# navallo/collision_avoidance

Measured on NVIDIA B200. Metric: orca_agent_steps_per_sec, higher is better.
Workload: dtype f32

## Files before the change

collision_avoidance_b200/build.py:

```python
from __future__ import annotations

import os
import shutil
import subprocess
import sys

PKG_DIR = os.path.dirname(os.path.abspath(__file__))
CSRC = os.path.join(PKG_DIR, "csrc")
LIB_PATH = os.path.join(PKG_DIR, "liborca_b200.so")

NVCC_FLAGS = [
    "-O3", "-std=c++17",
    "-gencode", "arch=compute_100a,code=sm_100a",
    "-lineinfo",
    "-fmad=false",
    "-Xcompiler", "-fPIC,-ffp-contract=off,-O2",
    "-shared",
]


def _sources_mtime() -> float:
    newest = 0.0
    for root in (CSRC, os.path.join(PKG_DIR, "..", "include")):
        for name in os.listdir(root):
            if name.endswith((".cu", ".cuh", ".h")):
                newest = max(newest, os.path.getmtime(os.path.join(root, name)))
    return newest


def nvcc_path() -> str:
    nvcc = shutil.which("nvcc") or "/usr/local/cuda/bin/nvcc"
    if not os.path.exists(nvcc):
        raise RuntimeError("nvcc not found: the CUDA library cannot be built")
    return nvcc


def build(force: bool = False, verbose: bool = False, extra_flags=()) -> str:
    if not force and os.path.exists(LIB_PATH) and os.path.getmtime(LIB_PATH) >= _sources_mtime():
        return LIB_PATH
    cmd = [nvcc_path(), *NVCC_FLAGS, *extra_flags, "-o", LIB_PATH, os.path.join(CSRC, "orca_api.cu")]
    if verbose:
        print(" ".join(cmd), file=sys.stderr)
    subprocess.check_call(cmd)
    return LIB_PATH


if __name__ == "__main__":
    flags = [a for a in sys.argv[1:] if a != "-v"]
    print(build(force=True, verbose=True, extra_flags=flags))
```

collision_avoidance_b200/csrc/orca_core.cuh:

```cuda
#pragma once

#include <math.h>
#include <stdint.h>

#if defined(__CUDACC__)
#define ORCA_HD __host__ __device__ __forceinline__
#define ORCA_HD_NOINLINE __host__ __device__ __noinline__
#else
#define ORCA_HD inline
#define ORCA_HD_NOINLINE inline
#include "host_vec_types.h"
#endif
#include <string.h>

#ifndef ORCA_MAX_OBST_NEIGHBORS
#define ORCA_MAX_OBST_NEIGHBORS 16
#endif
#ifndef ORCA_MAX_OBST_LINES
#define ORCA_MAX_OBST_LINES 6
#endif
#ifndef ORCA_MAX_ACTIONS
#define ORCA_MAX_ACTIONS 16
#endif
#define ORCA_MAX_BSP_DEPTH 64
#ifndef ORCA_SLOW_MAX_OBST
#define ORCA_SLOW_MAX_OBST 64
#endif

#if defined(ORCA_EMUL_COUNT) && !defined(__CUDA_ARCH__)
extern long long g_orca_counters[16];
#define ORCA_COUNT(slot, n) (g_orca_counters[slot] += (n))
#else
#define ORCA_COUNT(slot, n) ((void)0)
#endif

#if defined(ORCA_DEBUG_CHECKS)
#include <assert.h>
#define ORCA_DCHECK(cond) assert(cond)
#else
#define ORCA_DCHECK(cond) ((void)0)
#endif

namespace orca {

constexpr float kEps = 0.00001f;

ORCA_HD float bits_to_float(int i) {
#if defined(__CUDA_ARCH__)
  return __int_as_float(i);
#else
  float f;
  memcpy(&f, &i, 4);
  return f;
#endif
}
ORCA_HD int float_to_bits(float f) {
#if defined(__CUDA_ARCH__)
  return __float_as_int(f);
#else
  int i;
  memcpy(&i, &f, 4);
  return i;
#endif
}

ORCA_HD float2 v2(float x, float y) {
  float2 r;
  r.x = x;
  r.y = y;
  return r;
}
ORCA_HD float2 add(float2 a, float2 b) { return v2(a.x + b.x, a.y + b.y); }
ORCA_HD float2 sub(float2 a, float2 b) { return v2(a.x - b.x, a.y - b.y); }
ORCA_HD float2 neg(float2 a) { return v2(-a.x, -a.y); }
ORCA_HD float2 mul(float s, float2 a) { return v2(s * a.x, s * a.y); }
ORCA_HD float dot(float2 a, float2 b) { return a.x * b.x + a.y * b.y; }
ORCA_HD float det(float2 a, float2 b) { return a.x * b.y - a.y * b.x; }
ORCA_HD float abs_sq(float2 a) { return a.x * a.x + a.y * a.y; }
ORCA_HD float sqr(float s) { return s * s; }
ORCA_HD float2 div_s(float2 a, float s) {
  const float inv = 1.0f / s;
  return v2(a.x * inv, a.y * inv);
}
ORCA_HD float2 unit(float2 a) { return div_s(a, sqrtf(abs_sq(a))); }
ORCA_HD float left_of(float2 a, float2 b, float2 c) { return det(sub(a, c), sub(b, a)); }
ORCA_HD float fmin_first(float a, float b) { return (b < a) ? b : a; }
ORCA_HD float fmax_first(float a, float b) { return (a < b) ? b : a; }

ORCA_HD float dist_sq_point_segment(float2 a, float2 b, float2 c) {
  const float2 ab = sub(b, a);
  const float r = dot(sub(c, a), ab) / abs_sq(ab);
  if (r < 0.f) return abs_sq(sub(c, a));
  if (r > 1.f) return abs_sq(sub(c, b));
  return abs_sq(sub(c, add(a, mul(r, ab))));
}

struct Lines {
  float4* base;
  int stride;
  ORCA_HD float4 get(int i) const { return base[i * stride]; }
  ORCA_HD bool fetch(int i, float4& out) const {
    out = base[i * stride];
    return true;
  }
  ORCA_HD void set(int i, float2 point, float2 dir) const {
    float4 v;
    v.x = point.x;
    v.y = point.y;
    v.z = dir.x;
    v.w = dir.y;
    base[i * stride] = v;
  }
};
ORCA_HD float2 pt(float4 l) { return v2(l.x, l.y); }
ORCA_HD float2 dr(float4 l) { return v2(l.z, l.w); }

#if defined(__CUDA_ARCH__)
#define ORCA_LDG(p) __ldg(p)
#else
#define ORCA_LDG(p) (*(p))
#endif

struct ObstacleWorld {
  const float4* vert_pd;
  const int4* vert_link;
  const int4* bsp;
  const float4* bsp_seg;
  int n_nodes;
  const uint32_t* cull_rows;
  float4 cull_geo;
};

ORCA_HD bool obstacles_may_be_near(const ObstacleWorld& W, float2 p) {
  if (W.cull_rows == nullptr) return true;
  const float fx = (p.x - W.cull_geo.x) * W.cull_geo.z, fy = (p.y - W.cull_geo.y) * W.cull_geo.w;
  if (!(fx >= 0.f && fx < 32.f && fy >= 0.f && fy < 32.f)) return true;
  return ((ORCA_LDG(&W.cull_rows[(int)fy]) >> (int)fx) & 1u) != 0u;
}

#define ORCA_LD(p) (*(p))


template <class LS>
ORCA_HD bool lp1(const LS& S, int i, float4 li, float radius, float2 opt, bool dir_opt, float2& result) {
  const float2 pi = pt(li), di = dr(li);
  const float dp = dot(pi, di);
  const float disc = sqr(dp) + sqr(radius) - abs_sq(pi);
  if (disc < 0.f) return false;
  const float sq = sqrtf(disc);
  float t_lo = -dp - sq;
  float t_hi = -dp + sq;
  ORCA_COUNT(2, 1);
  ORCA_COUNT(3, i);
  for (int j = 0; j < i; ++j) {
    float4 lj;
    if (!S.fetch(j, lj)) continue;
    const float den = det(di, dr(lj));
    const float num = det(dr(lj), sub(pi, pt(lj)));
    if (fabsf(den) <= kEps) {
      if (num < 0.f) return false;
      continue;
    }
    const float t = num / den;
    if (den >= 0.f)
      t_hi = fmin_first(t_hi, t);
    else
      t_lo = fmax_first(t_lo, t);
    if (t_lo > t_hi) return false;
  }
  float t;
  if (dir_opt) {
    t = (dot(opt, di) > 0.f) ? t_hi : t_lo;
  } else {
    t = dot(di, sub(opt, pi));
    if (t < t_lo)
      t = t_lo;
    else if (t > t_hi)
      t = t_hi;
  }
  result = add(pi, mul(t, di));
  return true;
}

#if defined(__CUDA_ARCH__)
#define ORCA_ANY(mask, pred) __any_sync((mask), (pred))
#define ORCA_CONVERGE(mask) __syncwarp(mask)
#else
#define ORCA_ANY(mask, pred) (pred)
#define ORCA_CONVERGE(mask) ((void)0)
#endif

template <class LS>
ORCA_HD int lp2(unsigned mask, bool enabled, const LS& S, int n, float radius, float2 opt, bool dir_opt,
                float2& result) {
  if (dir_opt) {
    result = mul(radius, opt);
  } else if (abs_sq(opt) > sqr(radius)) {
    result = mul(radius, unit(opt));
  } else {
    result = opt;
  }
  int i = 0;
  int fail = n;
  bool active = enabled;
  while (ORCA_ANY(mask, active)) {
    float4 li;
    li.x = li.y = li.z = li.w = 0.f;
    if (active) {
      while (i < n) {
        if (S.fetch(i, li) && det(dr(li), sub(pt(li), result)) > 0.f) break;
        ++i;
      }
      active = i < n;
    }
    ORCA_CONVERGE(mask);
    if (active) {
      const float2 keep = result;
      if (!lp1(S, i, li, radius, opt, dir_opt, result)) {
        result = keep;
        fail = i;
        active = false;
      }
      ++i;
    }
  }
  return fail;
}

template <class LS>
struct ProjectedLines {
  LS L;
  float2 pi, di;
  int n_obst;
  ORCA_HD bool fetch(int j, float4& out) const {
    ORCA_COUNT(4, 1);
    const float4 lj = L.get(j);
    if (j < n_obst) {
      out = lj;
      return true;
    }
    const float2 pj = pt(lj), dj = dr(lj);
    const float d = det(di, dj);
    float2 np;
    if (fabsf(d) <= kEps) {
      if (dot(di, dj) > 0.f) return false;
      np = mul(0.5f, add(pi, pj));
    } else {
      np = add(pi, mul(det(dj, sub(pi, pj)) / d, di));
    }
    const float2 nd = unit(sub(dj, di));
    out.x = np.x;
    out.y = np.y;
    out.z = nd.x;
    out.w = nd.y;
    return true;
  }
};

template <class LS>
ORCA_HD void lp3(unsigned mask, bool need, const LS& L, int n, int n_obst, int begin, float radius, float2& result) {
  float distance = 0.f;
  int i = begin;
  bool active = need;
  while (ORCA_ANY(mask, active)) {
    ProjectedLines<LS> V;
    V.L = L;
    V.pi = v2(0.f, 0.f);
    V.di = v2(0.f, 0.f);
    V.n_obst = n_obst;
    if (active) {
      while (i < n) {
        const float4 li = L.get(i);
        V.pi = pt(li);
        V.di = dr(li);
        if (det(V.di, sub(V.pi, result)) > distance) break;
        ++i;
      }
      active = i < n;
      if (active) ORCA_COUNT(0, 1);
    }
    ORCA_CONVERGE(mask);
    const int m = active ? (i > n_obst ? i : n_obst) : 0;
    float2 cand = result;
    const int f = lp2(mask, active, V, m, radius, v2(-V.di.y, V.di.x), true, cand);
    if (active) {
      if (!(f < m)) result = cand;
      distance = det(V.di, sub(V.pi, result));
      ++i;
    }
  }
}

template <class LS, class PS>
ORCA_HD void lp3_stored(unsigned mask, bool need, const LS& L, int n, int n_obst, int begin, float radius, const PS& P,
                        float2& result) {
  float distance = 0.f;
  int i = begin;
  bool active = need;
  while (ORCA_ANY(mask, active)) {
    float2 pi = v2(0.f, 0.f), di = v2(0.f, 0.f);
    if (active) {
      while (i < n) {
        const float4 li = L.get(i);
        pi = pt(li);
        di = dr(li);
        if (det(di, sub(pi, result)) > distance) break;
        ++i;
      }
      active = i < n;
    }
    ORCA_CONVERGE(mask);
    int m = 0;
    if (active) {
      ProjectedLines<LS> V;
      V.L = L;
      V.pi = pi;
      V.di = di;
      V.n_obst = n_obst;
      const int hi = i > n_obst ? i : n_obst;
      for (int j = 0; j < hi; ++j) {
        float4 lj;
        if (V.fetch(j, lj)) P.set(m++, pt(lj), dr(lj));
      }
    }
    ORCA_CONVERGE(mask);
    float2 cand = result;
    const int f = lp2(mask, active, P, m, radius, v2(-di.y, di.x), true, cand);
    if (active) {
      if (!(f < m)) result = cand;
      distance = det(di, sub(pi, result));
      ++i;
    }
  }
}

ORCA_HD float4 agent_line(float2 p, float2 v, float2 po, float2 vo, float cr, float inv_th, float inv_dt,
                          bool* collided) {
  const float2 rp = sub(po, p);
  const float2 rv = sub(v, vo);
  const float d_sq = abs_sq(rp);
  const float cr_sq = sqr(cr);
  const bool apart = d_sq > cr_sq;
  const float inv_t = apart ? inv_th : inv_dt;
  const float2 w = sub(rv, mul(inv_t, rp));
  const float w_sq = abs_sq(w);
  const float dp1 = dot(w, rp);
  const bool on_circle = !apart || (dp1 < 0.f && sqr(dp1) > cr_sq * w_sq);
  const float root = sqrtf(on_circle ? w_sq : (d_sq - cr_sq));
  const float inv = 1.0f / (on_circle ? root : d_sq);
  float2 dir, u;
  if (on_circle) {
    const float2 uw = v2(w.x * inv, w.y * inv);
    dir = v2(uw.y, -uw.x);
    u = mul(cr * inv_t - root, uw);
  } else {
    const float leg = root;
    if (det(rp, w) > 0.f) {
      dir = v2((rp.x * leg - rp.y * cr) * inv, (rp.x * cr + rp.y * leg) * inv);
    } else {
      dir = neg(v2((rp.x * leg + rp.y * cr) * inv, (-rp.x * cr + rp.y * leg) * inv));
    }
    const float dp2 = dot(rv, dir);
    u = sub(mul(dp2, dir), rv);
  }
  *collided = !apart;
  const float2 point = add(v, mul(0.5f, u));
  float4 out;
  out.x = point.x;
  out.y = point.y;
  out.z = dir.x;
  out.w = dir.y;
  return out;
}

ORCA_HD unsigned lt_as_one_bits(float x, float y) {
#if defined(__CUDA_ARCH__)
  float one_or_zero;
  asm("set.lt.f32.f32 %0, %1, %2;" : "=f"(one_or_zero) : "f"(x), "f"(y));
  return __float_as_uint(one_or_zero);
#else
  return (x < y) ? 0x3f800000u : 0u;
#endif
}
ORCA_HD int one_bits_count(unsigned sum) { return (int)(((sum >> 23) * 383u) & 511u); }

template <int M>
ORCA_HD void rank_count(const float* d, int* r) {
#if defined(__CUDA_ARCH__)
  unsigned u[M];
#pragma unroll
  for (int j = 0; j < M; ++j) u[j] = (unsigned)j * 0x3f800000u;
#pragma unroll
  for (int i = 0; i < M; ++i) {
#pragma unroll
    for (int j = i + 1; j < M; ++j) {
      float j_first;
      asm("set.lt.f32.f32 %0, %1, %2;" : "=f"(j_first) : "f"(d[j]), "f"(d[i]));
      u[i] += __float_as_uint(j_first);
      u[j] -= __float_as_uint(j_first);
    }
  }
#pragma unroll
  for (int j = 0; j < M; ++j) r[j] = (int)(((u[j] >> 23) * 383u) & 511u);
#else
  for (int j = 0; j < M; ++j) r[j] = j;
  for (int i = 0; i < M; ++i) {
    for (int j = i + 1; j < M; ++j) {
      const int j_first = (d[j] < d[i]) ? 1 : 0;
      r[i] += j_first;
      r[j] -= j_first;
    }
  }
#endif
}

template <int K, bool KFULL>
struct NearestK {
  float d[K];
  int id[K];
  int k;
  float range_sq;
  uint4 packed;
  int packed_cnt;
  ORCA_HD void init(int k_, float range_sq_) {
    k = k_;
    range_sq = range_sq_;
    packed_cnt = -1;
#pragma unroll
    for (int s = 0; s < K; ++s) {
      d[s] = (KFULL || s < k) ? range_sq : -1.0f;
      id[s] = -1;
    }
  }
  ORCA_HD void set_sorted_ids(const uint4 packed_, int cnt) {
    packed = packed_;
    packed_cnt = cnt;
  }
  ORCA_HD void unpack_ids() {
#pragma unroll
    for (int s = 0; s < K; ++s) {
      const unsigned w = (s < 4) ? packed.x : (s < 8) ? packed.y : (s < 12) ? packed.z : packed.w;
      id[s] = (s < packed_cnt) ? (int)((w >> ((s & 3) * 8)) & 255u) : -1;
      d[s] = 0.f;
    }
  }
  ORCA_HD float thresh() const {
    if (KFULL) return d[K - 1];
    float m = d[0];
#pragma unroll
    for (int s = 1; s < K; ++s) m = fmaxf(m, d[s]);
    return m;
  }
  ORCA_HD void offer(float cand_d, int cand_id) {
    if (cand_d < thresh()) {
      bool prev_before = false;
      float prev_d = cand_d;
      int prev_i = cand_id;
#pragma unroll
      for (int s = 0; s < K; ++s) {
        const bool before = cand_d < d[s];
        const float old_d = d[s];
        const int old_i = id[s];
        d[s] = before ? (prev_before ? prev_d : cand_d) : old_d;
        id[s] = before ? (prev_before ? prev_i : cand_id) : old_i;
        prev_before = before;
        prev_d = old_d;
        prev_i = old_i;
      }
    }
  }
  ORCA_HD void finish() {}
  ORCA_HD bool full() const { return id[K - 1] >= 0; }
  ORCA_HD float kth_dist_sq() const { return d[K - 1]; }
  template <class Before>
  ORCA_HD void offer_ranked(float cand_d, int cand_id, const Before& precedes) {
    bool tie = false;
#pragma unroll
    for (int s = 0; s < K; ++s) tie = tie || (cand_d == d[s]);
    if (!tie) {
      offer(cand_d, cand_id);
      return;
    }
    if (cand_d <= thresh()) {
      bool prev_before = false;
      float prev_d = cand_d;
      int prev_i = cand_id;
#pragma unroll
      for (int s = 0; s < K; ++s) {
        bool before = cand_d < d[s];
        if (cand_d == d[s]) before = precedes(cand_id, id[s]);
        const float old_d = d[s];
        const int old_i = id[s];
        d[s] = before ? (prev_before ? prev_d : cand_d) : old_d;
        id[s] = before ? (prev_before ? prev_i : cand_id) : old_i;
        prev_before = before;
        prev_d = old_d;
        prev_i = old_i;
      }
    }
  }
};

template <int K, bool KFULL>
struct NearestKeys {
  unsigned long long key[K];
  int id[K];
  float d[K];
  int k;
  float range_sq;
  uint4 packed;
  int packed_cnt;
  ORCA_HD void init(int k_, float range_sq_) {
    k = k_;
    range_sq = range_sq_;
    packed_cnt = -1;
    const unsigned long long empty = (unsigned long long)(unsigned)float_to_bits(range_sq_) << 32;
#pragma unroll
    for (int s = 0; s < K; ++s) {
      key[s] = (KFULL || s < k) ? empty : 0ull;
      id[s] = -1;
      d[s] = 0.f;
    }
  }
  ORCA_HD float thresh() const {
    unsigned long long m = key[K - 1];
    if (!KFULL) {
#pragma unroll
      for (int s = 0; s < K - 1; ++s) m = key[s] > m ? key[s] : m;
    }
    return bits_to_float((int)(unsigned)(m >> 32));
  }
  ORCA_HD void offer(float cand_d, int cand_id) {
    unsigned long long x = ((unsigned long long)(unsigned)float_to_bits(cand_d) << 32) | (unsigned)(cand_id + 1);
    if (KFULL && !(x < key[K - 1])) return;
#pragma unroll
    for (int s = 0; s < K; ++s) {
      const unsigned long long cur = key[s];
      const bool in_front = x < cur;
      key[s] = in_front ? x : cur;
      x = in_front ? cur : x;
    }
  }
  template <class Before>
  ORCA_HD void offer_ranked(float cand_d, int cand_id, const Before&) {
    offer(cand_d, cand_id);
  }
  ORCA_HD void finish() {
#pragma unroll
    for (int s = 0; s < K; ++s) id[s] = (int)(unsigned)(key[s] & 0xffffffffull) - 1;
  }
  ORCA_HD bool full() const { return id[K - 1] >= 0; }
  ORCA_HD float kth_dist_sq() const { return bits_to_float((int)(unsigned)(key[K - 1] >> 32)); }
  ORCA_HD void pack_ids() {
    unsigned w[4] = {0u, 0u, 0u, 0u};
    int cnt = 0;
#pragma unroll
    for (int s = 0; s < K; ++s) {
      const bool valid = id[s] >= 0;
      w[s >> 2] |= valid ? ((unsigned)id[s] << ((s & 3) * 8)) : 0u;
      cnt += valid ? 1 : 0;
    }
    packed.x = w[0];
    packed.y = w[1];
    packed.z = w[2];
    packed.w = w[3];
    packed_cnt = cnt;
  }
  ORCA_HD void set_sorted_ids(const uint4 packed_, int cnt) {
    packed = packed_;
    packed_cnt = cnt;
  }
  ORCA_HD void unpack_ids() {
#pragma unroll
    for (int s = 0; s < K; ++s) {
      const unsigned w = (s < 4) ? packed.x : (s < 8) ? packed.y : (s < 12) ? packed.z : packed.w;
      id[s] = (s < packed_cnt) ? (int)((w >> ((s & 3) * 8)) & 255u) : -1;
    }
  }
};

#if defined(__CUDA_ARCH__)
#define ORCA_WARP_MAX(mask, v) __reduce_max_sync((mask), (v))
#else
#define ORCA_WARP_MAX(mask, v) (v)
#endif

struct CandidateBuffer {
  float4* base;
  int stride;
  int cap;
  int cnt;
  ORCA_HD float2* entry(int r) const { return reinterpret_cast<float2*>(&base[(r >> 1) * stride]) + (r & 1); }
  ORCA_HD void push(float d, int id) {
    ORCA_DCHECK(cnt >= 0 && cnt < cap);
    *entry(cnt) = v2(d, bits_to_float(id));
    ++cnt;
  }
  template <class Insert>
  ORCA_HD void drain(unsigned mask, const Insert& insert) {
    const int rounds = ORCA_WARP_MAX(mask, cnt);
    for (int r = 0; r < rounds; ++r) {
      if (r < cnt) {
        const float2 e = *entry(r);
        insert(e.x, float_to_bits(e.y));
      }
    }
    cnt = 0;
  }
  template <class Insert>
  ORCA_HD void drain_if_full(unsigned mask, const Insert& insert, int room = 1) {
    if (ORCA_ANY(mask, cnt + room > cap)) drain(mask, insert);
  }
};

template <int MAXN = ORCA_MAX_OBST_NEIGHBORS>
// ... 258 lines not shown
```

collision_avoidance_b200/csrc/orca_step_small.cuh:

```cuda
#pragma once

#include "orca_core.cuh"

namespace orca {

constexpr int kMaxDevices = 64;

enum : int { POLICY_EXTERNAL = 0, POLICY_GOAL = 1, POLICY_RL = 2, POLICY_ALAN = 3 };
enum : int { DONE_NONE = 0, DONE_GOAL_RADIUS = 1, DONE_X_BELOW = 2, DONE_GOAL_RADIUS_DEFERRED = 3 };
enum : int {
  STAT_AGENT_STEPS = 0,
  STAT_FINISHED = 1,
  STAT_COLLISIONS = 2,
  STAT_LP3_CALLS = 3,
  STAT_OVERFLOW = 4,
  STAT_SUM_ARRIVAL = 5,
  STAT_SUM_ARRIVAL2 = 6,
  STAT_SUM_REWARD = 7
};

struct StepArgs {
  int E, N, envs_per_block, env_base;
  int k;
  float dt, inv_dt, nd_sq, inv_th, inv_tho, radius, vmax, obst_range_sq;
// ... 472 lines not shown
        a.nbr_idx[(size_t)g * a.k + s] = (nk.id[s] >= 0) ? src.local_id(nk.id[s]) : -1;
        if (a.nbr_dsq != nullptr) a.nbr_dsq[(size_t)g * a.k + s] = (nk.id[s] >= 0) ? abs_sq(sub(p, src.pos(nk.id[s]))) : 0.f;
        cnt += (nk.id[s] >= 0) ? 1 : 0;
      }
    }
    a.nbr_cnt[g] = cnt;
  }
  if (a.onbr_idx != nullptr) {
    int* row = a.onbr_idx + (size_t)g * ORCA_MAX_OBST_NEIGHBORS;
    if ((reinterpret_cast<uintptr_t>(a.onbr_idx) & 15u) == 0u) {
#pragma unroll
      for (int s = 0; s < ORCA_MAX_OBST_NEIGHBORS; s += 4) {
        int4 w;
        w.x = (s + 0 < ocnt) ? oid[s + 0] : -1;
        w.y = (s + 1 < ocnt) ? oid[s + 1] : -1;
        w.z = (s + 2 < ocnt) ? oid[s + 2] : -1;
        w.w = (s + 3 < ocnt) ? oid[s + 3] : -1;
        *reinterpret_cast<int4*>(row + s) = w;
      }
    } else {
      for (int s = 0; s < ORCA_MAX_OBST_NEIGHBORS; ++s) row[s] = (s < ocnt) ? oid[s] : -1;
    }
    a.onbr_cnt[g] = ocnt;
  }
  if (a.neighbors_only) return false;

  int n_obst = 0;
  if (ocnt > 0)
    n_obst = obstacle_lines<OL>(W, p, v, HETERO ? ap.radius : a.radius, HETERO ? ap.inv_tho : a.inv_tho, od, oid, ocnt, L,
                                &overflow);
  const float inv_th = HETERO ? ap.inv_th : a.inv_th;
  int n = n_obst;
  unsigned collisions = 0;
  {
    const float cr = a.radius + a.radius;
#ifndef ORCA_UNROLLED_LINES
    if (nk.packed_cnt >= 0) {
      unsigned w0 = nk.packed.x, w1 = nk.packed.y, w2 = nk.packed.z, w3 = nk.packed.w;
      const int cnt = nk.packed_cnt;
#pragma unroll 1
      for (int s = 0; s < cnt; ++s) {
        const int j = (int)(w0 & 255u);
        w0 = (w0 >> 8) | (w1 << 24);
        w1 = (w1 >> 8) | (w2 << 24);
        w2 = (w2 >> 8) | (w3 << 24);
        w3 >>= 8;
        bool hit;
        ORCA_DCHECK(n < K + OL);
        const float4 ln = agent_line(p, v, src.pos(j), src.vel(j), HETERO ? ap.radius + src.radius(j) : cr, inv_th, a.inv_dt, &hit);
        L.base[n * L.stride] = ln;
        ++n;
        collisions += hit ? 1u : 0u;
      }
    } else {
      int ids[K + 1];
#pragma unroll
      for (int s = 0; s < K; ++s) ids[s] = nk.id[s];
      ids[K] = -1;
      int j = ids[0];
      float2 pj = v2(0.f, 0.f), vj = v2(0.f, 0.f);
      if (j >= 0) {
        pj = src.pos(j);
        vj = src.vel(j);
      }
#pragma unroll 1
      for (int s = 1; j >= 0; ++s) {
        const int jn = ids[s];
        float2 pn = pj, vn = vj;
        if (jn >= 0) {
          pn = src.pos(jn);
          vn = src.vel(jn);
        }
        bool hit;
        const float4 ln = agent_line(p, v, pj, vj, HETERO ? ap.radius + src.radius(j) : cr, inv_th, a.inv_dt, &hit);
        L.base[n * L.stride] = ln;
        ++n;
        collisions += hit ? 1u : 0u;
        j = jn;
        pj = pn;
        vj = vn;
      }
    }
#else
    {
      if (nk.packed_cnt >= 0) nk.unpack_ids();
#pragma unroll
      for (int s = 0; s < K; ++s) {
        const int j = nk.id[s];
        if (j >= 0) {
          bool hit;
          const float4 ln = agent_line(p, v, src.pos(j), src.vel(j), HETERO ? ap.radius + src.radius(j) : cr, inv_th, a.inv_dt, &hit);
          L.base[n * L.stride] = ln;
          ++n;
          collisions += hit ? 1u : 0u;
        }
      }
    }
#endif
  }
  c.n = n;
  c.n_obst = n_obst;
  c.collisions = collisions;
  c.overflow = overflow;

  c.fail = lp2(warp_mask, true, L, n, HETERO ? ap.vmax : a.vmax, pref, false, c.nv);
  return true;
}

struct SlowParams {
  int k;
  float nd_sq, inv_th, inv_tho, inv_dt, radius, vmax, obst_range_sq;
};
struct SlowResult {
  float2 nv;
  int n, n_obst, fail;
  unsigned collisions;
  bool overflow;
};
ORCA_HD SlowParams slow_params(const StepArgs& a) {
  SlowParams q;
  q.k = a.k;
  q.nd_sq = a.nd_sq;
  q.inv_th = a.inv_th;
  q.inv_tho = a.inv_tho;
  q.inv_dt = a.inv_dt;
  q.radius = a.radius;
  q.vmax = a.vmax;
  q.obst_range_sq = a.obst_range_sq;
  return q;
}
ORCA_HD SlowParams slow_params(const StepArgs& a, const float4* agent_params, const int g) {
  const AgentParams ap = load_agent_params(agent_params, g);
  SlowParams q;
  q.k = ap.k;
  q.nd_sq = ap.nd_sq;
  q.inv_th = ap.inv_th;
  q.inv_tho = ap.inv_tho;
  q.inv_dt = a.inv_dt;
  q.radius = ap.radius;
  q.vmax = ap.vmax;
  q.obst_range_sq = ap.obst_range_sq;
  return q;
}
template <int K, bool KFULL, class Src, bool HETERO = false>
ORCA_HD_NOINLINE SlowResult agent_slow_path(const SlowParams a, const Src src, const ObstacleWorld W, const Lines scratch,
                                            const int scratch_slots, const unsigned mask, const float2 p, const float2 v,
                                            const float2 pref) {
  bool overflow = false;
  float od[ORCA_SLOW_MAX_OBST];
  int oid[ORCA_SLOW_MAX_OBST];
  int ocnt = 0;
  obstacle_neighbors<ORCA_SLOW_MAX_OBST>(W, p, a.obst_range_sq, od, oid, &ocnt, &overflow);
  float4 buf[ORCA_SLOW_MAX_OBST + K];
  Lines L;
  L.base = buf;
  L.stride = 1;
  const int n_obst = obstacle_lines<ORCA_SLOW_MAX_OBST>(W, p, v, a.radius, a.inv_tho, od, oid, ocnt, L, &overflow);
  typename Src::template List<K, KFULL> nk;
  nk.init(a.k, a.nd_sq);
  src.gather(nk, p, scratch, scratch_slots, mask);
  if (nk.packed_cnt >= 0) nk.unpack_ids();
  int n = n_obst;
  unsigned collisions = 0;
  const float cr = a.radius + a.radius;
  for (int s = 0; s < K; ++s) {
    const int j = nk.id[s];
    if (j >= 0) {
      bool hit;
      buf[n++] = agent_line(p, v, src.pos(j), src.vel(j), HETERO ? a.radius + src.radius(j) : cr, a.inv_th, a.inv_dt, &hit);
      collisions += hit ? 1u : 0u;
    }
  }
  SlowResult r;
  r.n = n;
  r.n_obst = n_obst;
  r.collisions = collisions;
  r.overflow = overflow;
  r.nv = v2(0.f, 0.f);
  r.fail = lp2(mask, true, L, n, a.vmax, pref, false, r.nv);
  float2 nv = r.nv;
  lp3(mask, r.fail < n, L, n, n_obst, r.fail, a.vmax, nv);
  r.nv = nv;
  return r;
}
ORCA_HD void apply_slow_result(const SlowResult& r, AgentCarry& c) {
  c.nv = r.nv;
  c.n = r.n;
  c.n_obst = r.n_obst;
  c.fail = r.fail;
  c.collisions = r.collisions;
  c.overflow = r.overflow;
}

template <int POLICY>
ORCA_HD void agent_back(const StepArgs& a, const int env, const int la, const int g, const int estep,
                        const AgentCarry& c, const bool live = true) {
  stat_add_u64_warp(a.stats, STAT_AGENT_STEPS, live ? 1u : 0u);
  stat_add_u64_warp(a.stats, STAT_LP3_CALLS, (live && c.fail < c.n) ? 1u : 0u);

  const float2 v = c.nv;
  const float2 p = add(c.p, mul(a.dt, v));
  a.pos[g] = p;
  a.vel[g] = v;
  if (a.pos_mirror != nullptr) a.pos_mirror[g] = p;
  if (a.vel_mirror != nullptr) a.vel_mirror[g] = v;

  if (POLICY == POLICY_RL || POLICY == POLICY_ALAN) {
    const float r_goal = dot(v, c.gdir);
    const float r_polite = dot(v, c.pref);
    float R;
    if (POLICY == POLICY_RL)
      R = a.rl_scale * r_goal + (1.f - a.rl_scale) * r_polite;
    else
      R = a.alan_gamma * r_goal + (1.f - a.alan_gamma) * r_polite;
    if (a.reward != nullptr) a.reward[g] = R;
    stat_add_f64_warp(a.stats, STAT_SUM_REWARD, live ? R : 0.f);
    if (POLICY == POLICY_ALAN) {
      float* wrow = a.alan_w + (size_t)g * a.A;
      if (a.alan_window > 0 && ((estep + 1) % a.alan_window) == 0) {
        for (int i = 0; i < a.A; ++i) wrow[i] = 0.f;
      }
      wrow[c.act] = R;
    }
  }

  if (a.done_mode != DONE_NONE) {
    const uint8_t flag = a.done[g];
    if (flag == 2) {
      a.done[g] = 1;
      if (a.goal2 != nullptr) a.goal[g] = a.goal2[g];
    } else if (flag == 0) {
      bool hit;
      if (a.done_mode != DONE_X_BELOW) {
        const float2 d = sub(p, a.goal[g]);
        hit = sqrtf(abs_sq(d)) < 2.f * a.radius;
      } else {
        hit = p.x < a.done_x;
      }
      if (hit) {
        const bool defer = a.done_mode == DONE_GOAL_RADIUS_DEFERRED;
        a.done[g] = defer ? 2 : 1;
        const float t_arr = (float)(estep + 1) * a.dt;
        if (a.arrival != nullptr) a.arrival[g] = t_arr;
        if (a.goal2 != nullptr && !defer) a.goal[g] = a.goal2[g];
        if (a.env_done_cnt != nullptr) counter_inc(&a.env_done_cnt[env]);
        stat_add_u64(a.stats, STAT_FINISHED, 1ull);
        stat_add_f64(a.stats, STAT_SUM_ARRIVAL, (double)t_arr);
        stat_add_f64(a.stats, STAT_SUM_ARRIVAL2, (double)t_arr * (double)t_arr);
      }
    }
  }
  if (a.env_step != nullptr && la == 0 && !a.grid_path) a.env_step[env] = estep + 1;
  stat_add_u64_warp(a.stats, STAT_COLLISIONS, live ? c.collisions : 0u);
  stat_add_u64_warp(a.stats, STAT_OVERFLOW, c.overflow ? 1u : 0u);
}

template <int K, bool KFULL, int POLICY, bool HETERO = false, class Src>
ORCA_HD void agent_step_body(const StepArgs& a, const int env, const int la, const int g, float2 p, float2 v,
                             const int estep, const Src& src, const Lines L, const unsigned warp_mask,
                             const float4* agent_params = nullptr) {
  AgentCarry c;
  c.p = p;
  c.v = v;
  c.aim = (POLICY == POLICY_EXTERNAL) ? a.pref[g] : a.goal[g];
  const ObstacleWorld W = Src::kObstacleCull ? global_world_with_cull(a, env) : global_world(a, env);
  if (!agent_front<K, KFULL, POLICY, ORCA_MAX_OBST_LINES, HETERO>(a, env, g, estep, src, W, L, warp_mask, c, agent_params)) return;
  if (c.overflow)
    apply_slow_result(agent_slow_path<K, KFULL, Src, HETERO>(HETERO ? slow_params(a, agent_params, g) : slow_params(a), src, global_world(a, env), L,
                                                             K + ORCA_MAX_OBST_LINES, warp_mask, c.p, c.v, c.pref), c);
  else
    lp3(warp_mask, c.fail < c.n, L, c.n, c.n_obst, c.fail, HETERO ? load_agent_params(agent_params, g).vmax : a.vmax, c.nv);
  agent_back<POLICY>(a, env, la, g, estep, c);
}

#if defined(__CUDACC__)

#ifndef ORCA_STEP_MAX_THREADS
#define ORCA_STEP_MAX_THREADS 256
#endif
#ifndef ORCA_STEP_MIN_BLOCKS
#define ORCA_STEP_MIN_BLOCKS 3
#endif

#ifndef ORCA_LP3_SMEM_POOL
#define ORCA_LP3_SMEM_POOL 0
#endif
inline size_t step_smem_bytes(int K, int tpb, bool tile, int world_slots = 0, int obst_lines = ORCA_MAX_OBST_LINES,
                              bool hetero = false) {
  size_t b = (size_t)world_slots * 64 + 16;
  if (hetero) b += (size_t)tpb * (tile ? 8 : 4);
  b += (size_t)tpb * ((tile ? 16 : 0) + (size_t)(K + obst_lines) * 16 + 8 + 4 + 1) + 8 * 4;
#if ORCA_LP3_SMEM_POOL
  b += (size_t)(tpb / 2) * (K + obst_lines) * 16 + 16;
#endif
  return b;
}

#ifndef ORCA_BLOCK_LP3
#define ORCA_BLOCK_LP3 1
#endif
#ifndef ORCA_LP3_SMEM_POOL
#define ORCA_LP3_SMEM_POOL 0
#endif
template <int K, bool HETERO = false>
__device__ __forceinline__ void block_lp3(float4* s_lines, float4* s_pool, int* s_meta, float2* s_nv,
                                          unsigned char* s_queue, int* s_warp_cnt, const bool need, const AgentCarry& c, const float vmax,
                                          const bool area_was_borrowed = false, const float* s_vmax = nullptr) {
  const int tid = threadIdx.x, lane = tid & 31, warp = tid >> 5, nwarps = blockDim.x >> 5;
  if (area_was_borrowed) __syncthreads();
#if !ORCA_BLOCK_LP3
  {
    Lines L;
    L.base = s_lines + tid;
    L.stride = blockDim.x;
    float2 nv = c.nv;
    lp3(0xffffffffu, need, L, c.n, c.n_obst, c.fail, HETERO ? s_vmax[tid] : vmax, nv);
    s_nv[tid] = nv;
    __syncwarp();
    return;
  }
#endif
  s_meta[tid] = c.n | (c.n_obst << 8) | (c.fail << 16);
  s_nv[tid] = c.nv;
  const unsigned bal = __ballot_sync(0xffffffffu, need);
  if (lane == 0) s_warp_cnt[warp] = __popc(bal);
  __syncthreads();
  int offset = 0, total = 0;
  for (int w = 0; w < nwarps; ++w) {
    const int cw = s_warp_cnt[w];
    offset += (w < warp) ? cw : 0;
    total += cw;
  }
  {
    const unsigned below = (1u << lane) - 1u;
    if (need)
      s_queue[offset + __popc(bal & below)] = (unsigned char)tid;
    else
      s_queue[blockDim.x - 1 - ((warp << 5) - offset + __popc(~bal & below))] = (unsigned char)tid;
  }
  __syncthreads();
#if ORCA_LP3_SMEM_POOL
  const int pool = blockDim.x >> 1;
  for (int first = 0; first < total; first += pool) {
    if ((warp << 5) < pool && first + (warp << 5) < total) {
      const int slot = first + tid;
      const bool mine = slot < total;
      const int owner = mine ? (int)s_queue[slot] : tid;
      const int meta = s_meta[owner];
      Lines L;
      L.base = s_lines + owner;
      L.stride = blockDim.x;
      Lines P;
      P.base = s_pool + tid;
      P.stride = pool;
      float2 nv = s_nv[owner];
      lp3_stored(0xffffffffu, mine, L, meta & 0xff, (meta >> 8) & 0xff, (meta >> 16) & 0xff, HETERO ? s_vmax[owner] : vmax, P, nv);
      if (mine) s_nv[owner] = nv;
    }
  }
#else
  (void)s_pool;
  const int nfree = blockDim.x - total;
  int nstored = total < nfree ? total : nfree;
  if (nstored < total) nstored &= ~31;
  if ((warp << 5) < total) {
    const bool mine = tid < total;
    const int owner = mine ? (int)s_queue[tid] : tid;
    const int meta = s_meta[owner];
    Lines L;
    L.base = s_lines + owner;
    L.stride = blockDim.x;
    float2 nv = s_nv[owner];
    if ((warp << 5) < nstored) {
#if defined(ORCA_DEBUG_CHECKS)
      if (mine) {
        const int col = (int)s_queue[blockDim.x - 1 - tid];
        assert(col >= 0 && col < (int)blockDim.x && tid < nfree);
        for (int q = 0; q < total; ++q) assert((int)s_queue[q] != col);
        for (int q = 0; q < nstored; ++q) assert(q == tid || (int)s_queue[blockDim.x - 1 - q] != col);
        assert(owner >= 0 && owner < (int)blockDim.x && (meta & 0xff) <= K + ORCA_MAX_OBST_LINES);
        (void)K;
      }
#endif
      Lines P;
      P.base = s_lines + (mine ? (int)s_queue[blockDim.x - 1 - tid] : tid);
      P.stride = blockDim.x;
      lp3_stored(0xffffffffu, mine, L, meta & 0xff, (meta >> 8) & 0xff, (meta >> 16) & 0xff, HETERO ? s_vmax[owner] : vmax, P, nv);
    } else {
      lp3(0xffffffffu, mine, L, meta & 0xff, (meta >> 8) & 0xff, (meta >> 16) & 0xff, HETERO ? s_vmax[owner] : vmax, nv);
    }
    if (mine) s_nv[owner] = nv;
  }
#endif
  __syncthreads();
}

__device__ __forceinline__ int tile_float_to_ordered(float f) {
  const int i = __float_as_int(f);
  return i >= 0 ? i : i ^ 0x7fffffff;
}
__device__ __forceinline__ float tile_ordered_to_float(int i) { return __int_as_float(i >= 0 ? i : i ^ 0x7fffffff); }

template <class Src>
__device__ __forceinline__ void build_tile_grid(const StepArgs& a, void* area, const bool valid, const int le, const int la,
                                                const float2 p, Src& src) {
  const int tid = threadIdx.x, tpb = blockDim.x, lane = tid & 31, warp = tid >> 5, nwarps = tpb >> 5;
  const int envs = a.envs_per_block;
  int* cnt = reinterpret_cast<int*>(area);
  int* bbox = cnt + envs * kTileCells;
  unsigned short* start = reinterpret_cast<unsigned short*>(bbox + envs * 2);
  unsigned char* sorted = reinterpret_cast<unsigned char*>(start + envs * kTileStartStride);
  for (int i = tid; i < envs * kTileCells; i += tpb) cnt[i] = 0;
  if (tid < envs * 2) bbox[tid] = 0x7fffffff;
  __syncthreads();
  if (valid) {
    atomicMin(&bbox[2 * le], tile_float_to_ordered(p.x));
    atomicMin(&bbox[2 * le + 1], tile_float_to_ordered(p.y));
  }
  __syncthreads();
  int ck = 0, slot = 0, cx = 0, cy = 0;
  if (valid) {
    const float ox = tile_ordered_to_float(bbox[2 * le]), oy = tile_ordered_to_float(bbox[2 * le + 1]);
    cx = (int)floorf((p.x - ox) * a.tile_grid_inv_cell);
    cy = (int)floorf((p.y - oy) * a.tile_grid_inv_cell);
    cx = cx < 0 ? 0 : (cx >= kTileGrid ? kTileGrid - 1 : cx);
    cy = cy < 0 ? 0 : (cy >= kTileGrid ? kTileGrid - 1 : cy);
    ck = cy * kTileGrid + cx;
    slot = atomicAdd(&cnt[le * kTileCells + ck], 1);
  }
  __syncthreads();
  for (int e = warp; e < envs; e += nwarps) {
    const int c0 = cnt[e * kTileCells + 2 * lane], c1 = cnt[e * kTileCells + 2 * lane + 1];
    int incl = c0 + c1;
#pragma unroll
    for (int d = 1; d < 32; d <<= 1) {
      const int up = __shfl_up_sync(0xffffffffu, incl, d);
      if (lane >= d) incl += up;
    }
    const int excl = incl - (c0 + c1);
    start[e * kTileStartStride + 2 * lane] = (unsigned short)excl;
    start[e * kTileStartStride + 2 * lane + 1] = (unsigned short)(excl + c0);
    if (lane == 31) start[e * kTileStartStride + kTileCells] = (unsigned short)incl;
  }
  __syncthreads();
  ORCA_DCHECK(!valid || (start[le * kTileStartStride + ck] + slot < a.N && start[le * kTileStartStride + kTileCells] == a.N));
  ORCA_DCHECK((char*)(sorted + envs * a.N) - (char*)area <= 13 * (int)blockDim.x + 32);
  if (valid) sorted[le * a.N + start[le * kTileStartStride + ck] + slot] = (unsigned char)la;
  __syncthreads();
  src.cell_start = start + le * kTileStartStride;
  src.sorted = sorted + le * a.N;
  src.cx = cx;
  src.cy = cy;
  if (valid) {
    src.ox = tile_ordered_to_float(bbox[2 * le]);
    src.oy = tile_ordered_to_float(bbox[2 * le + 1]);
  }
}

template <int K, bool KFULL, int POLICY, int OL = ORCA_MAX_OBST_LINES, bool HETERO = false>
__global__ void __launch_bounds__(ORCA_STEP_MAX_THREADS, ((OL <= 2 || K <= 5) ? 4 : ORCA_STEP_MIN_BLOCKS)) step_small_kernel(const StepArgs a, const float4* __restrict__ agent_params) {
  extern __shared__ float4 smem4[];
  const int tpb = blockDim.x;
  float2* s_pos = reinterpret_cast<float2*>(smem4);
  float2* s_vel = s_pos + tpb;
  float4* s_lines = smem4 + tpb;
  float4* s_pool = s_lines + (K + OL) * tpb;
  float2* s_nv = reinterpret_cast<float2*>(s_pool + (ORCA_LP3_SMEM_POOL ? (K + OL) * (tpb / 2) : 0));
  int* s_meta = reinterpret_cast<int*>(s_nv + tpb);
  int* s_warp_cnt = s_meta + tpb;
  unsigned char* s_queue = reinterpret_cast<unsigned char*>(s_warp_cnt + 8);
  float4* s_world = reinterpret_cast<float4*>((reinterpret_cast<uintptr_t>(s_queue + tpb) + 15) & ~(uintptr_t)15);
  float* s_rad = reinterpret_cast<float*>(s_world + 4 * a.world_slots);
  float* s_vmax = s_rad + tpb;

  const int tid = threadIdx.x;
  const int N = a.N;
  const int le = tid / N;
  int la = tid - le * N;
  const int env0 = a.env_base + blockIdx.x * a.envs_per_block;
  const int env = env0 + le;
  const bool valid = (le < a.envs_per_block) && (env < a.E);
  int g = env * N + la;
  const bool tile_grid = !(OL <= 2) && a.tile_grid_inv_cell > 0.f;

  AgentCarry c;
  c.p = v2(0.f, 0.f);
  c.v = v2(0.f, 0.f);
  c.nv = v2(0.f, 0.f);
  c.n = c.n_obst = c.fail = 0;
  int estep = 0;
  bool env_live = true;
  c.aim = v2(0.f, 0.f);
  if (valid) {
    if (!a.neighbors_only && !tile_grid) c.aim = (POLICY == POLICY_EXTERNAL) ? a.pref[g] : a.goal[g];
    c.p = a.pos[g];
    c.v = a.vel[g];
    s_pos[tid] = c.p;
    s_vel[tid] = c.v;
    if (HETERO) s_rad[tid] = ORCA_LDG(&agent_params[2 * (size_t)g]).x;
    if (a.env_step != nullptr) estep = a.env_step[env];
    if (a.env_done_cnt != nullptr) env_live = a.env_done_cnt[env] < N;
  }
  const int slots = a.world_slots;
  if (slots > 0) {
    const size_t first = (size_t)env0 * a.vert_stride;
    const size_t limit = (a.vert_stride > 0) ? (size_t)a.E * a.vert_stride : (size_t)a.world_verts;
    for (int s = tid; s < slots; s += tpb) {
      if (first + s < limit) {
        s_world[s] = a.vert_pd[first + s];
        s_world[slots + s] = *reinterpret_cast<const float4*>(&a.vert_link[first + s]);
        s_world[2 * slots + s] = *reinterpret_cast<const float4*>(&a.bsp[first + s]);
        s_world[3 * slots + s] = a.bsp_seg[first + s];
      }
    }
  }
  __syncthreads();
  const unsigned warp_mask = __ballot_sync(0xffffffffu, valid);
  bool alive = valid;
  using Source = TileSourceT<(OL <= 2)>;
  Source src;
  if (tile_grid) {
    build_tile_grid(a, s_nv, valid, le, la, c.p, src);
    if (valid) {
      la = (int)src.sorted[la];
      g = env * N + la;
      c.p = s_pos[le * N + la];
      c.v = s_vel[le * N + la];
      int cx = (int)floorf((c.p.x - src.ox) * a.tile_grid_inv_cell);
      int cy = (int)floorf((c.p.y - src.oy) * a.tile_grid_inv_cell);
      src.cx = cx < 0 ? 0 : (cx >= kTileGrid ? kTileGrid - 1 : cx);
      src.cy = cy < 0 ? 0 : (cy >= kTileGrid ? kTileGrid - 1 : cy);
      if (!a.neighbors_only) c.aim = (POLICY == POLICY_EXTERNAL) ? a.pref[g] : a.goal[g];
    }
  }
  c.overflow = false;
  if (valid) {
    ObstacleWorld W = global_world(a, env);
    if (slots > 0) {
      const int off = le * a.vert_stride;
      W.vert_pd = s_world + off;
      W.vert_link = reinterpret_cast<const int4*>(s_world + slots) + off;
      W.bsp = reinterpret_cast<const int4*>(s_world + 2 * slots) + off;
      W.bsp_seg = s_world + 3 * slots + off;
    }
    Lines L;
    L.base = s_lines + tid;
    L.stride = tpb;
    src.env_pos = s_pos + le * N;
    src.env_vel = s_vel + le * N;
    src.n = N;
    src.self = la;
    src.full_range_sq = HETERO ? ORCA_LDG(&agent_params[2 * (size_t)g + 1]).x : a.nd_sq;
    if (HETERO) src.env_rad = s_rad + le * N;
    alive = agent_front<K, KFULL, POLICY, OL, HETERO>(a, env, g, estep, src, W, L, warp_mask, c, agent_params);
    if (HETERO) s_vmax[tid] = ORCA_LDG(&agent_params[2 * (size_t)g]).y;
  }
  if (a.neighbors_only) return;
  block_lp3<K, HETERO>(s_lines, s_pool, s_meta, s_nv, s_queue, s_warp_cnt, alive && !c.overflow && c.fail < c.n, c, a.vmax, tile_grid,
                       s_vmax);
  const unsigned slow_mask = __ballot_sync(0xffffffffu, alive && c.overflow);
  if (!alive) return;
  c.nv = s_nv[tid];
  if (c.overflow) {
    Lines L;
    L.base = s_lines + tid;
    L.stride = tpb;
    Source scan;
    scan.env_pos = s_pos + le * N;
    scan.env_vel = s_vel + le * N;
    scan.n = N;
    scan.self = la;
    if (HETERO) scan.env_rad = s_rad + le * N;
    apply_slow_result(agent_slow_path<K, KFULL, Source, HETERO>(HETERO ? slow_params(a, agent_params, g) : slow_params(a), scan, global_world(a, env), L,
                                                                K + OL, slow_mask, c.p, c.v, c.pref), c);
  }
  agent_back<POLICY>(a, env, la, g, estep, c, env_live);
}

#endif

}
```

Before: 4.665 billion.

## Spread lp3 line projection across warp lanes with prefix-sum work distribution

```diff
diff --git a/collision_avoidance_b200/build.py b/collision_avoidance_b200/build.py
--- a/collision_avoidance_b200/build.py
+++ b/collision_avoidance_b200/build.py
@@ -35,14 +35,14 @@
     return nvcc
 
 
-def build(force: bool = False, verbose: bool = False, extra_flags=()) -> str:
-    if not force and os.path.exists(LIB_PATH) and os.path.getmtime(LIB_PATH) >= _sources_mtime():
-        return LIB_PATH
-    cmd = [nvcc_path(), *NVCC_FLAGS, *extra_flags, "-o", LIB_PATH, os.path.join(CSRC, "orca_api.cu")]
+def build(force: bool = False, verbose: bool = False, extra_flags=(), out: str = LIB_PATH) -> str:
+    if not force and os.path.exists(out) and os.path.getmtime(out) >= _sources_mtime():
+        return out
+    cmd = [nvcc_path(), *NVCC_FLAGS, *extra_flags, "-o", out, os.path.join(CSRC, "orca_api.cu")]
     if verbose:
         print(" ".join(cmd), file=sys.stderr)
     subprocess.check_call(cmd)
-    return LIB_PATH
+    return out
 
 
 if __name__ == "__main__":
diff --git a/collision_avoidance_b200/csrc/orca_core.cuh b/collision_avoidance_b200/csrc/orca_core.cuh
--- a/collision_avoidance_b200/csrc/orca_core.cuh
+++ b/collision_avoidance_b200/csrc/orca_core.cuh
@@ -243,7 +243,10 @@
     const float d = det(di, dj);
     float2 np;
     if (fabsf(d) <= kEps) {
-      if (dot(di, dj) > 0.f) return false;
+      if (dot(di, dj) > 0.f) {
+        ORCA_COUNT(5, 1);
+        return false;
+      }
       np = mul(0.5f, add(pi, pj));
     } else {
       np = add(pi, mul(det(dj, sub(pi, pj)) / d, di));
@@ -291,7 +294,73 @@
   }
 }
 
-template <class LS, class PS>
+#if defined(__CUDA_ARCH__)
+__device__ __forceinline__ int project_round_lanes(unsigned mask, bool active, const Lines& L, const Lines& P, int i,
+                                                   int n_obst) {
+  const int lane = threadIdx.x & 31;
+  const int hi = active ? (i > n_obst ? i : n_obst) : 0;
+  int incl = hi;
+#pragma unroll
+  for (int d = 1; d < 32; d <<= 1) {
+    const int t = __shfl_up_sync(mask, incl, d);
+    if (lane >= d) incl += t;
+  }
+  const int total = __shfl_sync(mask, incl, 31);
+  const int first = incl - hi;
+  const int addr_l = (int)(size_t)L.base, addr_p = (int)(size_t)P.base;
+  int skipped = 0;
+  for (int base = 0; base < total; base += 32) {
+    const int item = base + lane;
+    int o = 0, first_o = 0;
+#pragma unroll
+    for (int step = 16; step > 0; step >>= 1) {
+      const int f = __shfl_sync(mask, first, o + step);
+      if (f <= item) {
+        o += step;
+        first_o = f;
+      }
+    }
+    const int dl = __shfl_sync(mask, addr_l, o) - addr_l;
+    const int dp = __shfl_sync(mask, addr_p, o) - addr_p;
+    const int packed = __shfl_sync(mask, i | (n_obst << 8) | (skipped << 16), o);
+    const bool valid = item < total;
+    const int j = item - first_o;
+    float4 lj;
+    bool exists = false;
+    if (valid) {
+      ProjectedLines<Lines> V;
+      V.L.base = reinterpret_cast<float4*>(reinterpret_cast<char*>(L.base) + dl);
+      V.L.stride = L.stride;
+      const float4 li = V.L.get(packed & 0xff);
+      V.pi = pt(li);
+      V.di = dr(li);
+      V.n_obst = (packed >> 8) & 0xff;
+      exists = V.fetch(j, lj);
+    }
+    const unsigned gone = __ballot_sync(mask, valid && !exists);
+    if (valid && exists) {
+      int slot = j - (packed >> 16);
+      if (gone != 0u) {
+        const int from = first_o > base ? first_o - base : 0;
+        slot -= __popc(gone & ((1u << lane) - 1u) & ~((1u << from) - 1u));
+      }
+      Lines Po;
+      Po.base = reinterpret_cast<float4*>(reinterpret_cast<char*>(P.base) + dp);
+      Po.stride = P.stride;
+      Po.set(slot, pt(lj), dr(lj));
+    }
+    if (gone != 0u && hi > 0) {
+      const int lo = first - base, up = first + hi - base;
+      const unsigned below_up = up >= 32 ? 0xffffffffu : (up <= 0 ? 0u : (1u << up) - 1u);
+      const unsigned below_lo = lo >= 32 ? 0xffffffffu : (lo <= 0 ? 0u : (1u << lo) - 1u);
+      skipped += __popc(gone & below_up & ~below_lo);
+    }
+  }
+  return hi - skipped;
+}
+#endif
+
+template <bool LANES = true, class LS, class PS>
 ORCA_HD void lp3_stored(unsigned mask, bool need, const LS& L, int n, int n_obst, int begin, float radius, const PS& P,
                         float2& result) {
   float distance = 0.f;
@@ -311,6 +380,11 @@
     }
     ORCA_CONVERGE(mask);
     int m = 0;
+#if defined(__CUDA_ARCH__) && !defined(ORCA_LP3_SERIAL_PROJ)
+    if (LANES) {
+      m = project_round_lanes(mask, active, L, P, i, n_obst);
+    } else
+#endif
     if (active) {
       ProjectedLines<LS> V;
       V.L = L;
diff --git a/collision_avoidance_b200/csrc/orca_step_small.cuh b/collision_avoidance_b200/csrc/orca_step_small.cuh
--- a/collision_avoidance_b200/csrc/orca_step_small.cuh
+++ b/collision_avoidance_b200/csrc/orca_step_small.cuh
@@ -798,7 +798,7 @@
 #ifndef ORCA_LP3_SMEM_POOL
 #define ORCA_LP3_SMEM_POOL 0
 #endif
-template <int K, bool HETERO = false>
+template <int K, bool HETERO = false, bool LANES = true>
 __device__ __forceinline__ void block_lp3(float4* s_lines, float4* s_pool, int* s_meta, float2* s_nv,
                                           unsigned char* s_queue, int* s_warp_cnt, const bool need, const AgentCarry& c, const float vmax,
                                           const bool area_was_borrowed = false, const float* s_vmax = nullptr) {
@@ -881,7 +881,8 @@
       Lines P;
       P.base = s_lines + (mine ? (int)s_queue[blockDim.x - 1 - tid] : tid);
       P.stride = blockDim.x;
-      lp3_stored(0xffffffffu, mine, L, meta & 0xff, (meta >> 8) & 0xff, (meta >> 16) & 0xff, HETERO ? s_vmax[owner] : vmax, P, nv);
+      lp3_stored<LANES>(0xffffffffu, mine, L, meta & 0xff, (meta >> 8) & 0xff, (meta >> 16) & 0xff, HETERO ? s_vmax[owner] : vmax, P,
+                        nv);
     } else {
       lp3(0xffffffffu, mine, L, meta & 0xff, (meta >> 8) & 0xff, (meta >> 16) & 0xff, HETERO ? s_vmax[owner] : vmax, nv);
     }
@@ -1052,8 +1053,8 @@
     if (HETERO) s_vmax[tid] = ORCA_LDG(&agent_params[2 * (size_t)g]).y;
   }
   if (a.neighbors_only) return;
-  block_lp3<K, HETERO>(s_lines, s_pool, s_meta, s_nv, s_queue, s_warp_cnt, alive && !c.overflow && c.fail < c.n, c, a.vmax, tile_grid,
-                       s_vmax);
+  block_lp3<K, HETERO, POLICY != POLICY_ALAN>(s_lines, s_pool, s_meta, s_nv, s_queue, s_warp_cnt, alive && !c.overflow && c.fail < c.n, c,
+                                               a.vmax, tile_grid, s_vmax);
   const unsigned slow_mask = __ballot_sync(0xffffffffu, alive && c.overflow);
   if (!alive) return;
   c.nv = s_nv[tid];
```

Result: faster. 4.804 billion, median of 6 (+3.0%).
